# SinOncology/BreakID

Hardware: AMD Instinct MI355X
Metric: M reads/s clustered+split-scanned (higher is better)
Workload: dtype int32/u8 (+f64 sd replay)

## Files before the change

breakid_amd/csrc/lanes.hip:

```cpp
#include <algorithm>
#include <atomic>
#include <chrono>
#include <cmath>
#include <cstdio>
#include <numeric>
#include <thread>
#include <dirent.h>

#include "lanes.h"

static int g_hw_queues_at_init = 0;
void stage_set_hw_queues(int n) { g_hw_queues_at_init = n; }

static bool sort_service_on()
{
  static const bool on = !(getenv("BREAKID_SORT_SERVICE") && atoi(getenv("BREAKID_SORT_SERVICE")) == 0);
  return on;
}
constexpr int LANE_STREAMS_MAX = 4;
constexpr int SVC_STAGE_QUEUES = LANE_STREAMS_MAX + 3;
static bool lane_service(int fast) { return sort_service_on() && fast && g_hw_queues_at_init >= SVC_STAGE_QUEUES; }
static int stage_queues() { return std::max(1, g_hw_queues_at_init - 1); }
static int lanes_wanted(bool svc)
{
  const char *env = getenv("BREAKID_GROUP_LANES");
  static const int want_svc = env ? atoi(env) : 12;
  if (svc) return want_svc < 1 ? 1 : (want_svc > 26 ? 26 : want_svc);
  static const int want = env ? atoi(env) : std::min(4, stage_queues());
  return want < 1 ? 1 : (want > 26 ? 26 : want);
}
static bool lanes_apply(const StageInput &in, int fast)
{
  static const uint64_t min_pairs = getenv("BREAKID_LANES_MIN_PAIRS") ? strtoull(getenv("BREAKID_LANES_MIN_PAIRS"), nullptr, 10) : (1ull << 20);
  uint32_t large = 0;
  const uint64_t big = std::max<uint64_t>(2, min_pairs >> 6);
  for (uint32_t g = 0; g < in.jr.n_groups && g + 1 < in.gstart_host.size(); ++g) large += in.gstart_host[g + 1] - in.gstart_host[g] >= big ? 1u : 0u;
  const bool yes = lanes_wanted(lane_service(fast)) >= 2 && fast && in.jr.n_groups >= 4 && in.jr.n_pairs >= min_pairs && large >= 2;
  if (yes)
  {
    static bool told = false;
    const int K = lanes_wanted(lane_service(fast));
    if (!told && !lane_service(fast) && K > stage_queues() && bk_debug("lanes"))
    {
      told = true;
      fprintf(stderr, "[breakid] GPU_MAX_HW_QUEUES=%d: the lanes of chromosome-pair groups (bk_mask_and_cluster) and their heap kernels will share hardware queues "
                        "(BREAKID_GROUP_LANES=1: one pass)\n", g_hw_queues_at_init);
    }
  }
  return yes;
}

__global__ void k_svc_probe() {}
static int kfd_compute_queues(int device)
{
  char bus[64] = {0};
  if (hipDeviceGetPCIBusId(bus, (int) sizeof bus, device) != hipSuccess) return -1;
  unsigned dom = 0, b = 0, d = 0, f = 0;
  if (sscanf(bus, "%x:%x:%x.%x", &dom, &b, &d, &f) != 4) return -1;
  const unsigned long want_loc = (b << 8) | (d << 3) | f;
  auto read_file = [](const std::string &path, std::string &out) {
    FILE *fp = fopen(path.c_str(), "r");
    if (!fp) return false;
    char buf[4096];
    const size_t n = fread(buf, 1, sizeof buf - 1, fp);
    fclose(fp);
    buf[n] = 0;
    out = buf;
    return true;
  };
  auto list_dir = [](const std::string &path, std::vector<std::string> &names) {
    DIR *dp = opendir(path.c_str());
    if (!dp) return false;
    while (dirent *e = readdir(dp))
      if (e->d_name[0] != '.') names.push_back(e->d_name);
    closedir(dp);
    return true;
  };
  unsigned long gpu_id = 0;
  {
    std::vector<std::string> nodes;
    if (!list_dir("/sys/class/kfd/kfd/topology/nodes", nodes)) return -1;
    for (const std::string &n : nodes)
    {
      std::string props, id;
      const std::string base = "/sys/class/kfd/kfd/topology/nodes/" + n;
      if (!read_file(base + "/properties", props) || !read_file(base + "/gpu_id", id)) continue;
      unsigned long loc = ~0ul, domain = ~0ul;
      size_t p = props.find("location_id ");
      if (p != std::string::npos) loc = strtoul(props.c_str() + p + 12, nullptr, 10);
      p = props.find("domain ");
      if (p != std::string::npos) domain = strtoul(props.c_str() + p + 7, nullptr, 10);
      if (loc == want_loc && (domain == ~0ul || domain == dom) && strtoul(id.c_str(), nullptr, 10) != 0) gpu_id = strtoul(id.c_str(), nullptr, 10);
    }
  }
  if (!gpu_id) return -1;
  std::vector<std::string> procs;
  if (!list_dir("/sys/class/kfd/kfd/proc", procs)) return -1;
  int total = 0;
  for (const std::string &pid : procs)
  {
    std::vector<std::string> qs;
    const std::string qdir = "/sys/class/kfd/kfd/proc/" + pid + "/queues";
    if (!list_dir(qdir, qs)) continue;
    for (const std::string &q : qs)
    {
      std::string g, t;
      if (!read_file(qdir + "/" + q + "/gpuid", g) || !read_file(qdir + "/" + q + "/type", t)) continue;
      if (strtoul(g.c_str(), nullptr, 10) == gpu_id && strtoul(t.c_str(), nullptr, 10) == 0) ++total;
    }
  }
  return total;
}
constexpr int SVC_MAX_DEVICE_QUEUES = 24;
static std::mutex g_svc_device_m[64];
static void tell_no_service()
{
  static std::atomic<bool> told{false};
  if (!getenv("BREAKID_QUIET") && !told.exchange(true))
    fprintf(stderr, "[breakid] the resident sort service shares a hardware queue with a stream of its own stage (GPU_MAX_HW_QUEUES too low for the streams of this process), or other processes hold hardware queues on this device: sorting by launches instead\n");
}
struct SvcStage
{
  ClusterStage &cs;
  hipStream_t st;
  bool on;
  std::unique_lock<std::mutex> device_turn;
  SvcStage(ClusterStage &s, int device, hipStream_t st, bool want, uint64_t n_bound, uint64_t max_group, const std::vector<hipStream_t> &streams)
      : cs(s), st(st), on(want && sort_service_on() && !s.svc_refused)
  {
    if (on && device >= 0 && device < 64)
    {
      device_turn = std::unique_lock<std::mutex>(g_svc_device_m[device], std::try_to_lock);
      on = device_turn.owns_lock();
    }
    if (!on) return;
    const auto ts0 = std::chrono::steady_clock::now();
    cs.svc.start(n_bound, max_group + 2, st);
    const auto ts1 = std::chrono::steady_clock::now();
    int census;
    {
      static std::mutex cm;
      static std::chrono::steady_clock::time_point when[64];
      static int last[64];
      static bool have[64] = {};
      std::lock_guard<std::mutex> l(cm);
      const int d = device & 63;
      if (!have[d] || std::chrono::duration<double>(ts1 - when[d]).count() > 0.25)
      {
        last[d] = kfd_compute_queues(device);
        when[d] = std::chrono::steady_clock::now();
        have[d] = true;
      }
      census = last[d];
    }
    if (bk_debug("lanes"))
      fprintf(stderr, "[lanes] sort service started in %.3f ms; compute queues on the device (all processes): %d (counted in %.3f ms)\n", std::chrono::duration<double, std::milli>(ts1 - ts0).count(), census,
              std::chrono::duration<double, std::milli>(std::chrono::steady_clock::now() - ts1).count());
    const bool crowded = census > SVC_MAX_DEVICE_QUEUES;
    const bool behind = !crowded && !reachable(streams);
    const bool late = !crowded && !behind && !cs.svc.narrow_running(0.03);
    if (crowded || behind || late)
    {
      cs.svc.stop();
      on = false;
      if (crowded || behind || ++cs.svc_late >= 2) cs.svc_refused = true;
      device_turn.unlock();
      tell_no_service();
      return;
    }
    cs.svc_late = 0;
    set(&cs.svc);
  }
  bool reachable(const std::vector<hipStream_t> &streams)
  {
    while (cs.svc_probe.size() < streams.size())
    {
      hipEvent_t e;
      HIP_CHECK(hipEventCreateWithFlags(&e, hipEventDisableTiming));
      cs.svc_probe.push_back(e);
    }
    for (size_t k = 0; k < streams.size(); ++k)
    {
      hipLaunchKernelGGL(k_svc_probe, dim3(1), dim3(64), 0, streams[k]);
      HIP_CHECK(hipEventRecord(cs.svc_probe[k], streams[k]));
    }
    const auto t0 = std::chrono::steady_clock::now();
    auto since = [&] { return std::chrono::duration<double>(std::chrono::steady_clock::now() - t0).count(); };
    bool ok = true;
    for (size_t k = 0; k < streams.size() && ok; ++k)
      for (;;)
      {
        const hipError_t e = hipEventQuery(cs.svc_probe[k]);
        if (e == hipSuccess) break;
        if (e != hipErrorNotReady) throw bk_error(BK_ERR_HIP, std::string("sort service probe: ") + hipGetErrorString(e));
        if (since() > 0.05)
        {
          ok = false;
          break;
        }
      }
    const double took = since();
    if (bk_debug("lanes")) fprintf(stderr, "[lanes] sort service probe: %zu streams in %.3f ms%s\n", streams.size(), took * 1e3, ok ? "" : " (gave up)");
    return ok && took < 0.003;
  }
  void set(SortService *s)
  {
    for (auto &l : cs.lanes)
    {
      l->cb.se.svc = s;
      l->cb.se.svc_slot = 0xFFFFFFFFu;
    }
  }
  void finish()
  {
    if (!on) return;
    on = false;
    set(nullptr);
    hipError_t e = hipStreamSynchronize(st);
    for (auto &l : cs.lanes)
      if (l->st && e == hipSuccess) e = hipStreamSynchronize(l->st);
    cs.svc.stop();
    device_turn.unlock();
    if (e != hipSuccess) throw bk_error(BK_ERR_HIP, std::string("sort service: ") + hipGetErrorString(e));
  }
  ~SvcStage()
  {
    try
    {
      finish();
    }
    catch (const bk_error &)
    {
    }
  }
};

static void snapshot_list(const PairList &L, DevBuf &idx, DevBuf *gof, DevBuf &goff, hipStream_t st)
{
  uint32_t *ii = idx.as<uint32_t>(L.n + 1), *ig = gof ? gof->as<uint32_t>(L.n + 1) : nullptr;
  uint64_t *io = goff.as<uint64_t>((uint64_t) L.ng + 1);
  if (L.n) HIP_CHECK(hipMemcpyAsync(ii, L.idx.get<uint32_t>(), L.n * 4, hipMemcpyDeviceToDevice, st));
  if (L.n && ig) HIP_CHECK(hipMemcpyAsync(ig, L.gof.get<uint32_t>(), L.n * 4, hipMemcpyDeviceToDevice, st));
  if (L.ng) HIP_CHECK(hipMemcpyAsync(io, L.goff.get<uint64_t>(), ((uint64_t) L.ng + 1) * 8, hipMemcpyDeviceToDevice, st));
}
static void cluster_list(const bk_pair *pairs, PairList &L, double w, int fast, DevBuf &cl, ClusterBufs &cb, AhcBufs &ab, hipStream_t st)
{
  if (fast)
    fast_cluster_all(pairs, L, w, cl, cb, st);
  else
    ahc_cluster_all(pairs, L, w, cl, ab, cb, st);
}

using LanePlan = std::vector<int>;
static LanePlan plan_owned(const StageInput &in)
{
  const uint32_t ng = in.jr.n_groups;
  const bool owned_only = !in.own_groups.empty();
  if (owned_only && in.own_groups.size() != ng) throw bk_error(BK_ERR_ARG, "bk_shard_own_groups: group count changed");
  LanePlan p(ng, 0);
  for (uint32_t g = 0; owned_only && g < ng; ++g)
    if (!in.own_groups[g]) p[g] = -1;
  return p;
}
static LanePlan plan_blind(const StageInput &in, int K)
{
  const uint32_t ng = in.jr.n_groups;
  std::vector<uint32_t> order(ng);
  std::iota(order.begin(), order.end(), 0u);
  auto size_of = [&](uint32_t g) { return in.gstart_host[g + 1] - in.gstart_host[g]; };
  std::stable_sort(order.begin(), order.end(), [&](uint32_t a, uint32_t b) { return size_of(a) > size_of(b); });
  constexpr double wexp = 2.0;
  LanePlan p = plan_owned(in);
  std::vector<double> load(K, 0.0);
  for (uint32_t i = 0; i < ng; ++i)
  {
    const uint32_t g = order[i];
    if (p[g] < 0) continue;
    int l = 0;
    for (int k = 1; k < K; ++k)
      if (load[k] < load[l]) l = k;
    load[l] += std::pow((double) size_of(g), wexp);
    p[g] = l;
  }
  return p;
}
static LanePlan plan_observed(const std::vector<uint64_t> &sizes, const std::vector<uint32_t> &hx, const std::vector<uint32_t> &hy, int K)
{
  const uint32_t ng = (uint32_t) sizes.size();
  constexpr double per_pair = 0.001;
  auto heap_cost = [](uint32_t m) { return (double) m + (m > 40947u ? 1.0 * (double) (m - 40947u) : 0.0); };
  std::vector<uint32_t> order(ng);
  std::iota(order.begin(), order.end(), 0u);
  auto chain = [&](uint32_t g) { return heap_cost(hx[g]) + heap_cost(hy[g]); };
  std::stable_sort(order.begin(), order.end(), [&](uint32_t a, uint32_t b) {
    const double ca = chain(a), cb = chain(b);
    return ca != cb ? ca > cb : sizes[a] > sizes[b];
  });
  LanePlan p(ng, 0);
  std::vector<double> mx(K, 0.0), my(K, 0.0), pairs(K, 0.0);
  auto cost = [&](int l) { return mx[l] + my[l] + per_pair * pairs[l]; };
  for (uint32_t g : order)
  {
    int best = 0;
    double best_cost = 0;
    for (int l = 0; l < K; ++l)
    {
      const double c = std::max(mx[l], heap_cost(hx[g])) + std::max(my[l], heap_cost(hy[g])) + per_pair * (pairs[l] + (double) sizes[g]);
      if (l == 0 || c < best_cost || (c == best_cost && cost(l) < cost(best)))
      {
        best = l;
        best_cost = c;
      }
    }
    mx[best] = std::max(mx[best], heap_cost(hx[g]));
    my[best] = std::max(my[best], heap_cost(hy[g]));
    pairs[best] += (double) sizes[g];
    p[g] = best;
  }
  if (bk_debug("lanes"))
    for (int l = 0; l < K; ++l)
    {
      fprintf(stderr, "[lanes] lane %d: max heap x %.0f y %.0f, %.0f pairs, cost %.0f; heavy groups:", l, mx[l], my[l], pairs[l], cost(l));
      for (uint32_t g = 0; g < ng; ++g)
        if (p[g] == l && (hx[g] || hy[g])) fprintf(stderr, " %u(%u,%u)", g, hx[g], hy[g]);
      fprintf(stderr, "\n");
    }
  return p;
}
static uint32_t *upload_drop(const LanePlan &p, int K, DevBuf &buf, hipStream_t st)
{
  const size_t row = p.size() + 1;
  std::vector<uint32_t> drop((size_t) K * row, 0u);
  for (int l = 0; l < K; ++l)
    for (size_t g = 0; g + 1 < row; ++g) drop[(size_t) l * row + g] = p[g] == l ? 0u : 1u;
  uint32_t *d = buf.as<uint32_t>(drop.size() + 1);
  HIP_CHECK(hipMemcpyAsync(d, drop.data(), drop.size() * 4, hipMemcpyHostToDevice, st));
  HIP_CHECK(hipStreamSynchronize(st));
  return d;
}

static void group_lanes(ClusterStage &cs, const StageInput &in, double w, int fast)
{
  const uint32_t ng = in.jr.n_groups;
  static const bool dbg = bk_debug("lanes");
  auto make_lanes = [&](int K, int S) {
    while ((int) cs.lanes.size() < K)
    {
      cs.lanes.emplace_back(new ClusterStage::Lane());
      cs.lanes.back()->cb.max_group_bound = cs.cb().max_group_bound;
    }
    for (int k = 1; k < S; ++k)
      if (!cs.lanes[k]->st) HIP_CHECK(hipStreamCreateWithFlags(&cs.lanes[k]->st, hipStreamNonBlocking));
  };
  bool use_svc = sort_service_on() && fast;
  if (use_svc && !lane_service(fast))
  {
    use_svc = false;
    tell_no_service();
    if (bk_debug("lanes")) fprintf(stderr, "[lanes] %d hardware queues, the sort service needs %d: not started\n", g_hw_queues_at_init, SVC_STAGE_QUEUES);
  }
  int K = lanes_wanted(use_svc);
  int S = use_svc ? std::max(1, std::min(LANE_STREAMS_MAX, K)) : K;
  make_lanes(K, S);
  std::vector<hipStream_t> stage_streams{in.st};
  for (int k = 1; k < S; ++k) stage_streams.push_back(cs.lanes[k]->st);
  SvcStage svc_stage(cs, in.device, in.st, use_svc, in.jr.n_pairs + 2ull * ng + 4096, cs.cb().max_group_bound, stage_streams);
  if (use_svc && !svc_stage.on)
  {
    use_svc = false;
    K = lanes_wanted(false);
    S = K;
    make_lanes(K, S);
  }
  if (!use_svc && bk_debug("lanes"))
  {
    fprintf(stderr, "[lanes] launch path: %d lanes, 1 stream each, %d hardware queues\n", K, g_hw_queues_at_init);
    fprintf(stderr, "[lanes] sorts as task dispatches on the lane streams\n");
  }
  auto lane = [&](int l) -> ClusterStage::Lane & { return *cs.lanes[l]; };
  auto lane_st = [&](int l) { const int k = l % S; return k == 0 ? in.st : cs.lanes[k]->st; };
  uint32_t *drop_base = nullptr;
  auto lane_drop = [&](int l) { return drop_base + (size_t) l * ((size_t) ng + 1); };
  std::vector<std::vector<uint8_t>> keep(K, std::vector<uint8_t>(ng, 0));
  auto upload_plan = [&](const LanePlan &p) {
    for (int l = 0; l < K; ++l)
      for (uint32_t g = 0; g < ng; ++g) keep[l][g] = p[g] == l ? 1 : 0;
    drop_base = upload_drop(p, K, cs.d_drop, in.st);
  };
  auto in_lanes = [&](auto body) {
    std::vector<std::string> err(K);
    std::vector<int> code(K, BK_OK);
    const auto t_start = std::chrono::steady_clock::now();
    auto guarded_body = [&](int l) {
      try
      {
        body(l);
        HIP_CHECK(hipStreamSynchronize(lane_st(l)));
        if (dbg)
          fprintf(stderr, "[lanes] lane %d done after %.2f ms\n", l, std::chrono::duration<double, std::milli>(std::chrono::steady_clock::now() - t_start).count());
      }
      catch (const bk_error &e)
      {
        code[l] = e.code;
        err[l] = e.msg;
      }
    };
    std::vector<std::thread> th;
    for (int l = 1; l < K; ++l)
      th.emplace_back([&, l] {
        (void) hipSetDevice(in.device);
        guarded_body(l);
      });
    guarded_body(0);
    for (std::thread &t : th) t.join();
    for (int l = 0; l < K; ++l)
      if (code[l] != BK_OK) throw bk_error(code[l], err[l]);
  };
  auto merge_all = [&](PairList ClusterStage::Lane::*which, PairList &out, DevBuf *cl_out) {
    std::vector<const PairList *> ls(K);
    std::vector<const uint32_t *> cls(K);
    for (int l = 0; l < K; ++l)
    {
      ls[l] = &(lane(l).*which);
      cls[l] = lane(l).d_cluster.get<uint32_t>();
    }
    merge_lists_many(ls.data(), cl_out ? cls.data() : nullptr, K, out, cl_out, in.st);
  };
  const bk_pair *pairs = in.jr.pairs;
  auto mask_lane = [&](int l, bool observe) {
    ClusterBufs &cb = lane(l).cb;
    if (observe)
    {
      cb.heavy_x.assign(ng, 0u);
      cb.heavy_y.assign(ng, 0u);
      cb.observe = true;
      cb.se.heavy_all = false;
    }
    remove_isolated_begin(pairs, in.jr.gof, in.jr.gstart, ng, in.jr.n_pairs, w, lane(l).list, cb, lane_st(l), lane_drop(l), in.gstart_host.data(), keep[l].data());
    if (observe) cb.heavy_x.assign(ng, 0u);
    remove_isolated_end(pairs, lane(l).list, cb, lane_st(l));
    if (observe) cb.observe = false;
  };
  auto cluster_lane = [&](int l) {
    PairList &L = lane(l).list, &iso = lane(l).iso;
    iso.n = L.n;
    iso.ng = L.ng;
    snapshot_list(L, iso.idx, &iso.gof, iso.goff, lane_st(l));
    cluster_list(pairs, L, w, fast, lane(l).d_cluster, lane(l).cb, cs.ab, lane_st(l));
  };
  const auto tp0 = std::chrono::steady_clock::now();
  auto phase = [&](const char *what) {
    if (dbg) fprintf(stderr, "[lanes] %s at %.2f ms\n", what, std::chrono::duration<double, std::milli>(std::chrono::steady_clock::now() - tp0).count());
  };
  upload_plan(plan_blind(in, K));
  phase("plan uploaded");
  if (use_svc)
    in_lanes([&](int l) {
      mask_lane(l, false);
      cluster_lane(l);
    });
  else
  {
    in_lanes([&](int l) { mask_lane(l, true); });
    PairList &mid = cs.lane_mid;
    merge_all(&ClusterStage::Lane::list, mid, nullptr);
    std::vector<uint64_t> goff_h((size_t) ng + 1);
    HIP_CHECK(hipMemcpyAsync(goff_h.data(), mid.goff.get<uint64_t>(), ((size_t) ng + 1) * 8, hipMemcpyDeviceToHost, in.st));
    HIP_CHECK(hipStreamSynchronize(in.st));
    std::vector<uint64_t> sizes(ng);
    std::vector<uint32_t> hx(ng, 0u), hy(ng, 0u);
    for (uint32_t g = 0; g < ng; ++g) sizes[g] = goff_h[g + 1] - goff_h[g];
    for (int l = 0; l < K; ++l)
      for (uint32_t g = 0; g < ng; ++g)
      {
        hx[g] = std::max(hx[g], lane(l).cb.heavy_x[g]);
        hy[g] = std::max(hy[g], lane(l).cb.heavy_y[g]);
      }
    upload_plan(plan_observed(sizes, hx, hy, K));
    in_lanes([&](int l) {
      list_subset_ranges(mid, goff_h.data(), keep[l].data(), lane(l).list, lane_st(l));
      cluster_lane(l);
    });
  }
  phase("lanes done");
  svc_stage.finish();
  phase("service stopped");
  if (use_svc && bk_debug("lanes")) fprintf(stderr, "[svc] tasks: %u wide, %u narrow\n", cs.svc.stats[0], cs.svc.stats[1]);
  PairList &iso_m = cs.lane_iso_m;
  merge_all(&ClusterStage::Lane::iso, iso_m, nullptr);
  merge_all(&ClusterStage::Lane::list, cs.list, &cs.d_cluster);
  HIP_CHECK(hipStreamSynchronize(in.st));
  phase("lists merged");
  cs.iso_n = iso_m.n;
  std::swap(cs.iso_idx, iso_m.idx);
  std::swap(cs.iso_goff, iso_m.goff);
}

void ClusterStage::run(const StageInput &in, double w, int fast)
{
  uint64_t mg = 0;
  for (uint32_t g = 0; g < in.jr.n_groups && g + 1 < in.gstart_host.size(); ++g) mg = std::max<uint64_t>(mg, in.gstart_host[g + 1] - in.gstart_host[g]);
  for (auto &l : lanes) l->cb.max_group_bound = mg;
  if (lanes_apply(in, fast))
  {
    in.timed("mask_and_cluster_lanes", [&] { group_lanes(*this, in, w, fast); });
    return;
  }
  SvcStage svc_stage(*this, in.device, in.st, true, in.jr.n_pairs + 2ull * in.jr.n_groups + 4096, cb().max_group_bound, {in.st});
  in.timed("remove_isolated", [&] {
    const uint32_t *drop = in.own_groups.empty() ? nullptr : upload_drop(plan_owned(in), 1, d_drop, in.st);
    remove_isolated_all(in.jr.pairs, in.jr.gof, in.jr.gstart, in.jr.n_groups, in.jr.n_pairs, w, list, cb(), in.st, drop);
  });
  iso_n = list.n;
  snapshot_list(list, iso_idx, nullptr, iso_goff, in.st);
  if (!fast) svc_stage.finish();
  in.timed(fast ? "fast_cluster" : "ahc_cluster", [&] { cluster_list(in.jr.pairs, list, w, fast, d_cluster, cb(), ab, in.st); });
  svc_stage.finish();
}

void ClusterStage::sort_forms(uint64_t out[3]) const
{
  out[0] = out[1] = out[2] = 0;
  for (const auto &l : lanes)
    for (int k = 0; k < 2; ++k) out[k] += l->cb.se.sorts[k];
}

void ClusterStage::debug_sort(int device, hipStream_t st, uint32_t *key, uint32_t *idx, const uint32_t *gof, const uint64_t *goff, uint32_t ng, uint64_t n, uint64_t max_group)
{
  SvcStage svc_stage(*this, device, st, true, n + 2ull * ng + 4096, max_group, {st});
  std_sort_groups(key, idx, gof, goff, ng, n, cb().se, st);
  svc_stage.finish();
}
```

Measured before the change: 11740.

## Plan lane assignment with a cost model and local search

Replaces the greedy heap-cost lane planner with a model-based planner. It seeds from the greedy plan, runs swap/move local search over heavy groups to minimise a modelled per-lane makespan, then places light groups greedily under the same model. The seed plan is kept unless the model predicts an improvement. This adds host planning time, and its benefit rests on how well the fitted model constants match the real lane timings.

Result: faster. 12170 (median of 6 runs) (+3.6%).

```diff
diff --git a/breakid_amd/csrc/lane_plan.h b/breakid_amd/csrc/lane_plan.h
--- /dev/null
+++ b/breakid_amd/csrc/lane_plan.h
@@ -0,0 +1,212 @@
+#pragma once
+#include <algorithm>
+#include <cstdint>
+#include <numeric>
+#include <vector>
+
+namespace lane_plan
+{
+using Plan = std::vector<int>;
+
+constexpr uint32_t HEAVY_MIN = 4096;
+constexpr uint32_t LDS_ENTRIES = 40947;
+constexpr int MAX_HEAVY = 64;
+constexpr int MAX_EVALS = 4000;
+
+inline double heap_cost(uint32_t m) { return (double) m + (m > LDS_ENTRIES ? (double) (m - LDS_ENTRIES) : 0.0); }
+
+struct Model
+{
+  double t_spine = 1.1;
+  double c_pop = 0.178e-3;
+  double t_part0 = 0.35, t_part1 = 0.455e-6;
+  double t_small0 = 1.37, t_small1 = 0.31e-6;
+};
+
+struct Lane
+{
+  uint32_t hx = 0, hy = 0;
+  double pairs = 0.0;
+};
+inline double lane_time(const Model &m, const Lane &l)
+{
+  const double part = m.t_part0 + m.t_part1 * l.pairs;
+  return std::max(m.t_spine + m.c_pop * heap_cost(l.hx), part) + std::max(m.t_spine + m.c_pop * heap_cost(l.hy), part) + m.t_small0 + m.t_small1 * l.pairs;
+}
+struct Objective
+{
+  double makespan = 0.0, sum = 0.0;
+  bool operator<(const Objective &o) const { return makespan != o.makespan ? makespan < o.makespan : sum < o.sum; }
+};
+inline std::vector<Lane> lanes_of(const Plan &p, const std::vector<uint64_t> &sizes, const std::vector<uint32_t> &hx, const std::vector<uint32_t> &hy, int K)
+{
+  std::vector<Lane> L((size_t) K);
+  for (size_t g = 0; g < p.size(); ++g)
+  {
+    if (p[g] < 0 || p[g] >= K) continue;
+    Lane &l = L[(size_t) p[g]];
+    l.hx = std::max(l.hx, hx[g]);
+    l.hy = std::max(l.hy, hy[g]);
+    l.pairs += (double) sizes[g];
+  }
+  return L;
+}
+inline Objective objective(const Model &m, const std::vector<Lane> &L)
+{
+  Objective o;
+  for (const Lane &l : L)
+  {
+    const double t = lane_time(m, l);
+    o.makespan = std::max(o.makespan, t);
+    o.sum += t;
+  }
+  return o;
+}
+inline Objective evaluate(const Model &m, const Plan &p, const std::vector<uint64_t> &sizes, const std::vector<uint32_t> &hx, const std::vector<uint32_t> &hy, int K)
+{
+  return objective(m, lanes_of(p, sizes, hx, hy, K));
+}
+
+inline Plan plan_greedy(const std::vector<uint64_t> &sizes, const std::vector<uint32_t> &hx, const std::vector<uint32_t> &hy, int K)
+{
+  const uint32_t ng = (uint32_t) sizes.size();
+  constexpr double per_pair = 0.001;
+  std::vector<uint32_t> order(ng);
+  std::iota(order.begin(), order.end(), 0u);
+  auto chain = [&](uint32_t g) { return heap_cost(hx[g]) + heap_cost(hy[g]); };
+  std::stable_sort(order.begin(), order.end(), [&](uint32_t a, uint32_t b) {
+    const double ca = chain(a), cb = chain(b);
+    return ca != cb ? ca > cb : sizes[a] > sizes[b];
+  });
+  Plan p(ng, 0);
+  std::vector<double> mx((size_t) K, 0.0), my((size_t) K, 0.0), pairs((size_t) K, 0.0);
+  auto cost = [&](int l) { return mx[l] + my[l] + per_pair * pairs[l]; };
+  for (uint32_t g : order)
+  {
+    int best = 0;
+    double best_cost = 0;
+    for (int l = 0; l < K; ++l)
+    {
+      const double c = std::max(mx[l], heap_cost(hx[g])) + std::max(my[l], heap_cost(hy[g])) + per_pair * (pairs[l] + (double) sizes[g]);
+      if (l == 0 || c < best_cost || (c == best_cost && cost(l) < cost(best)))
+      {
+        best = l;
+        best_cost = c;
+      }
+    }
+    mx[best] = std::max(mx[best], heap_cost(hx[g]));
+    my[best] = std::max(my[best], heap_cost(hy[g]));
+    pairs[best] += (double) sizes[g];
+    p[g] = best;
+  }
+  return p;
+}
+
+struct Stats
+{
+  int heavy = 0, evals = 0, moves = 0;
+  bool improved = false;
+  Objective seed, result;
+};
+
+inline Plan plan_model(const std::vector<uint64_t> &sizes, const std::vector<uint32_t> &hx, const std::vector<uint32_t> &hy, int K, const Model &m = Model(), Stats *stats = nullptr)
+{
+  const uint32_t ng = (uint32_t) sizes.size();
+  const Plan seed = plan_greedy(sizes, hx, hy, K);
+  Stats s;
+  s.seed = s.result = evaluate(m, seed, sizes, hx, hy, K);
+  ++s.evals;
+  std::vector<uint32_t> heavy, light;
+  for (uint32_t g = 0; g < ng; ++g) (hx[g] >= HEAVY_MIN || hy[g] >= HEAVY_MIN ? heavy : light).push_back(g);
+  s.heavy = (int) heavy.size();
+  auto done = [&](const Plan &p) {
+    if (stats) *stats = s;
+    return p;
+  };
+  if (K < 2 || heavy.empty() || (int) heavy.size() > MAX_HEAVY) return done(seed);
+
+  Plan p(ng, -1);
+  for (uint32_t g : heavy) p[g] = seed[g];
+  auto lanes_without = [&](const Plan &q) { return lanes_of(q, sizes, hx, hy, K); };
+  Objective cur = objective(m, lanes_without(p));
+  ++s.evals;
+  for (bool better = true; better && s.evals < MAX_EVALS;)
+  {
+    better = false;
+    Objective best = cur;
+    uint32_t bg = 0, bh = 0;
+    int bl = -1;
+    auto consider = [&](uint32_t g, uint32_t h, int l) {
+      const Objective o = objective(m, lanes_without(p));
+      ++s.evals;
+      if (o < best)
+      {
+        best = o;
+        bg = g;
+        bh = h;
+        bl = l;
+      }
+    };
+    for (size_t i = 0; i < heavy.size() && s.evals < MAX_EVALS; ++i)
+    {
+      const uint32_t g = heavy[i];
+      const int from = p[g];
+      for (int l = 0; l < K && s.evals < MAX_EVALS; ++l)
+      {
+        if (l == from) continue;
+        p[g] = l;
+        consider(g, g, l);
+      }
+      p[g] = from;
+      for (size_t j = i + 1; j < heavy.size() && s.evals < MAX_EVALS; ++j)
+      {
+        const uint32_t h = heavy[j];
+        if (p[h] == from) continue;
+        std::swap(p[g], p[h]);
+        consider(g, h, -2);
+        std::swap(p[g], p[h]);
+      }
+    }
+    if (bl == -1) break;
+    if (bl >= 0)
+      p[bg] = bl;
+    else
+      std::swap(p[bg], p[bh]);
+    cur = best;
+    better = true;
+    ++s.moves;
+  }
+
+  std::stable_sort(light.begin(), light.end(), [&](uint32_t a, uint32_t b) { return sizes[a] > sizes[b]; });
+  std::vector<Lane> L = lanes_without(p);
+  for (uint32_t g : light)
+  {
+    int bl = 0;
+    Objective best;
+    for (int l = 0; l < K; ++l)
+    {
+      const Lane keep = L[(size_t) l];
+      L[(size_t) l].hx = std::max(keep.hx, hx[g]);
+      L[(size_t) l].hy = std::max(keep.hy, hy[g]);
+      L[(size_t) l].pairs += (double) sizes[g];
+      const Objective o = objective(m, L);
+      L[(size_t) l] = keep;
+      if (l == 0 || o < best)
+      {
+        best = o;
+        bl = l;
+      }
+    }
+    p[g] = bl;
+    L[(size_t) bl].hx = std::max(L[(size_t) bl].hx, hx[g]);
+    L[(size_t) bl].hy = std::max(L[(size_t) bl].hy, hy[g]);
+    L[(size_t) bl].pairs += (double) sizes[g];
+  }
+  const Objective fin = evaluate(m, p, sizes, hx, hy, K);
+  ++s.evals;
+  if (!(fin < s.seed)) return done(seed);
+  s.result = fin;
+  s.improved = true;
+  return done(p);
+}
+}
diff --git a/breakid_amd/csrc/lanes.hip b/breakid_amd/csrc/lanes.hip
--- a/breakid_amd/csrc/lanes.hip
+++ b/breakid_amd/csrc/lanes.hip
@@ -8,6 +8,7 @@
 #include <dirent.h>
 
 #include "lanes.h"
+#include "lane_plan.h"
 
 static int g_hw_queues_at_init = 0;
 void stage_set_hw_queues(int n) { g_hw_queues_at_init = n; }
@@ -287,44 +288,35 @@
 static LanePlan plan_observed(const std::vector<uint64_t> &sizes, const std::vector<uint32_t> &hx, const std::vector<uint32_t> &hy, int K)
 {
   const uint32_t ng = (uint32_t) sizes.size();
-  constexpr double per_pair = 0.001;
-  auto heap_cost = [](uint32_t m) { return (double) m + (m > 40947u ? 1.0 * (double) (m - 40947u) : 0.0); };
-  std::vector<uint32_t> order(ng);
-  std::iota(order.begin(), order.end(), 0u);
-  auto chain = [&](uint32_t g) { return heap_cost(hx[g]) + heap_cost(hy[g]); };
-  std::stable_sort(order.begin(), order.end(), [&](uint32_t a, uint32_t b) {
-    const double ca = chain(a), cb = chain(b);
-    return ca != cb ? ca > cb : sizes[a] > sizes[b];
-  });
-  LanePlan p(ng, 0);
-  std::vector<double> mx(K, 0.0), my(K, 0.0), pairs(K, 0.0);
-  auto cost = [&](int l) { return mx[l] + my[l] + per_pair * pairs[l]; };
-  for (uint32_t g : order)
-  {
-    int best = 0;
-    double best_cost = 0;
+  static const bool greedy_only = getenv("BREAKID_LANE_PLAN") && std::string(getenv("BREAKID_LANE_PLAN")) == "greedy";
+  const auto t0 = std::chrono::steady_clock::now();
+  lane_plan::Stats stats;
+  const lane_plan::Model model;
+  const LanePlan p = greedy_only ? lane_plan::plan_greedy(sizes, hx, hy, K) : lane_plan::plan_model(sizes, hx, hy, K, model, &stats);
+  const double plan_ms = std::chrono::duration<double, std::milli>(std::chrono::steady_clock::now() - t0).count();
+  if (bk_debug("lanes"))
+  {
+    const std::vector<lane_plan::Lane> L = lane_plan::lanes_of(p, sizes, hx, hy, K);
     for (int l = 0; l < K; ++l)
     {
-      const double c = std::max(mx[l], heap_cost(hx[g])) + std::max(my[l], heap_cost(hy[g])) + per_pair * (pairs[l] + (double) sizes[g]);
-      if (l == 0 || c < best_cost || (c == best_cost && cost(l) < cost(best)))
-      {
-        best = l;
-        best_cost = c;
-      }
-    }
-    mx[best] = std::max(mx[best], heap_cost(hx[g]));
-    my[best] = std::max(my[best], heap_cost(hy[g]));
-    pairs[best] += (double) sizes[g];
-    p[g] = best;
-  }
-  if (bk_debug("lanes"))
-    for (int l = 0; l < K; ++l)
-    {
-      fprintf(stderr, "[lanes] lane %d: max heap x %.0f y %.0f, %.0f pairs, cost %.0f; heavy groups:", l, mx[l], my[l], pairs[l], cost(l));
+      const double mx = lane_plan::heap_cost(L[l].hx), my = lane_plan::heap_cost(L[l].hy);
+      fprintf(stderr, "[lanes] lane %d: max heap x %.0f y %.0f, %.0f pairs, cost %.0f; heavy groups:", l, mx, my, L[l].pairs, mx + my + 0.001 * L[l].pairs);
       for (uint32_t g = 0; g < ng; ++g)
         if (p[g] == l && (hx[g] || hy[g])) fprintf(stderr, " %u(%u,%u)", g, hx[g], hy[g]);
       fprintf(stderr, "\n");
     }
+    for (int l = 0; l < K; ++l)
+    {
+      uint32_t groups = 0;
+      for (uint32_t g = 0; g < ng; ++g) groups += p[g] == l ? 1u : 0u;
+      fprintf(stderr, "[lanes] lane %d: %u groups, modelled %.2f ms\n", l, groups, lane_plan::lane_time(model, L[l]));
+    }
+    if (greedy_only)
+      fprintf(stderr, "[lanes] part 2 plan: greedy (BREAKID_LANE_PLAN), planned in %.3f ms on the host\n", plan_ms);
+    else
+      fprintf(stderr, "[lanes] part 2 plan: model, %d heavy groups, %d evaluations, %d steps, makespan %.2f ms (seed %.2f ms)%s, planned in %.3f ms on the host\n", stats.heavy, stats.evals, stats.moves,
+              stats.result.makespan, stats.seed.makespan, stats.improved ? "" : ": the seed stays", plan_ms);
+  }
   return p;
 }
 static uint32_t *upload_drop(const LanePlan &p, int K, DevBuf &buf, hipStream_t st)
```
